# HugoVuach/Dense-linear-app

Measured on AMD Instinct MI355X. Metric: fp64 TFLOP/s for NxN SPD Cholesky (N^3/3 flops / factorisation time), higher is better.
Workload: dtype f64

## Files before the change

dense_linear_app_amd/csrc/kernels.hip:

```cpp
#include "cholmi_internal.h"

#include <type_traits>

#if defined(__HIP_DEVICE_COMPILE__) && !defined(__gfx950__)
#error "libcholmi's kernels target gfx950 (MI355X) only: build with --offload-arch=gfx950"
#endif

namespace cholmi {

typedef double d4_t __attribute__((ext_vector_type(4)));
typedef double d2_t __attribute__((ext_vector_type(2)));
typedef float f4_t __attribute__((ext_vector_type(4)));

template <typename T>
struct Tr;
template <>
struct Tr<double> {
  using acc_t = d4_t;
  using vec_t = d2_t;
  static constexpr int EPV = 2;
  static __device__ __forceinline__ acc_t mfma(double a, double b, acc_t c) {
    return __builtin_amdgcn_mfma_f64_16x16x4f64(a, b, c, 0, 0, 0);
  }
  static __device__ __forceinline__ int drow(int lane, int reg) { return (lane >> 4) + 4 * reg; }
// ... 84 lines not shown
  __syncthreads();
  const int nk = K / BK;
  for (int kt = 0; kt < nk; ++kt) {
    const int cur = kt & 1;
    if (kt + 1 < nk) gload((kt + 1) * BK);
    T af[4], bf[4];
#pragma unroll
    for (int ks = 0; ks < BK / 4; ++ks) {
      const int kk = ks * 4 + (lane >> 4);
#pragma unroll
      for (int a = 0; a < 4; ++a) af[a] = sm.a[cur][kk][wr * 64 + a * 16 + (lane & 15)];
#pragma unroll
      for (int b = 0; b < 4; ++b) bf[b] = sm.b[cur][kk][wc * 64 + b * 16 + (lane & 15)];
      if (ks == BK / 4 - 1 && kt + 1 < nk) lstore(cur ^ 1);
#pragma unroll
      for (int a = 0; a < 4; ++a)
#pragma unroll
        for (int b = 0; b < 4; ++b) acc[a][b] = Tr<T>::mfma(bf[b], af[a], acc[a][b]);
    }
    __syncthreads();
  }
}

__device__ __forceinline__ int cu_slot() {
  const unsigned hw = __builtin_amdgcn_s_getreg(4 | (0 << 6) | (31 << 11));
  const unsigned xcc = __builtin_amdgcn_s_getreg(20 | (0 << 6) | (3 << 11));
  return (int)(((((xcc & 7u) * 8u + ((hw >> 13) & 7u)) * 2u + ((hw >> 12) & 1u)) * 16u) + ((hw >> 8) & 15u));
}
struct GuestOnCu {
  int *slot;
  __device__ __forceinline__ explicit GuestOnCu(int *tab) : slot(nullptr) {
    if (tab) {
      slot = tab + cu_slot();
      if (threadIdx.x == 0) __hip_atomic_fetch_add(slot, 1, __ATOMIC_RELAXED, __HIP_MEMORY_SCOPE_AGENT);
    }
  }
  __device__ __forceinline__ void leave() {
    if (slot && threadIdx.x == 0) __hip_atomic_fetch_add(slot, -1, __ATOMIC_RELAXED, __HIP_MEMORY_SCOPE_AGENT);
  }
};
__device__ __forceinline__ void yield_to_guest(const int *slot) {
  for (int spin = 0; spin < 4000; ++spin) {
    if (__hip_atomic_load(slot, __ATOMIC_RELAXED, __HIP_MEMORY_SCOPE_AGENT) == 0) break;
    __builtin_amdgcn_s_sleep(20);
  }
}

__device__ __forceinline__ void sem_wait(const int *sem, int target, int *fail) {
  if (sem) {
    if (threadIdx.x == 0) {
      bool ok = false;
      for (int i = 0; i < (1 << 25); ++i) {
        if (__hip_atomic_load(sem, __ATOMIC_RELAXED, __HIP_MEMORY_SCOPE_AGENT) >= target) {
          ok = true;
          break;
        }
        __builtin_amdgcn_s_sleep(8);
      }
      __builtin_amdgcn_fence(__ATOMIC_ACQUIRE, "agent");
      asm volatile("s_waitcnt vmcnt(0)" ::: "memory");
      if (!ok && fail) atomicExch(fail, 0x7ffffffe);
    }
    __syncthreads();
  }
}
__device__ __forceinline__ void sem_signal(int *sem) {
  if (sem) {
    __syncthreads();
    if (threadIdx.x == 0) {
      __builtin_amdgcn_fence(__ATOMIC_RELEASE, "agent");
      asm volatile("s_waitcnt vmcnt(0)" ::: "memory");
      __hip_atomic_fetch_add(sem, 1, __ATOMIC_RELAXED, __HIP_MEMORY_SCOPE_AGENT);
    }
  }
}

__device__ __forceinline__ double load_sc1(const double *p) { return __hip_atomic_load(p, __ATOMIC_RELAXED, __HIP_MEMORY_SCOPE_AGENT); }
__device__ __forceinline__ float load_sc1(const float *p) { return __hip_atomic_load(p, __ATOMIC_RELAXED, __HIP_MEMORY_SCOPE_AGENT); }
__device__ __forceinline__ void store_sc1(double *p, double v) { __hip_atomic_store(p, v, __ATOMIC_RELAXED, __HIP_MEMORY_SCOPE_AGENT); }
__device__ __forceinline__ void store_sc1(float *p, float v) { __hip_atomic_store(p, v, __ATOMIC_RELAXED, __HIP_MEMORY_SCOPE_AGENT); }
__device__ __forceinline__ void store_pair_sc1(double *p, double a, double b) {
  d2_t v = {a, b};
  asm volatile("global_store_dwordx4 %0, %1, off sc1" ::"v"(p), "v"(v) : "memory");
}
__device__ __forceinline__ void store_pair_sc1(float *p, float a, float b) {
  typedef float f2_t __attribute__((ext_vector_type(2)));
  f2_t v = {a, b};
  asm volatile("global_store_dwordx2 %0, %1, off sc1" ::"v"(p), "v"(v) : "memory");
}

__device__ __forceinline__ void dbg_mark(unsigned long long *dbg, int tag, int step, unsigned long long t0) {
  if (dbg && threadIdx.x == 0) {
    const unsigned long long slot = atomicAdd(dbg, 1ull);
    if (slot < 1000) {
      unsigned long long *p = dbg + 1 + 8 * slot;
      p[0] = t0;
      p[1] = __builtin_amdgcn_s_memrealtime();
      p[2] = (unsigned long long)tag;
      p[3] = (unsigned long long)step;
    }
  }
}

__global__ void k_sem_probe_wait(const int *sem, int *result) {
  int ok = 2;
  for (int i = 0; i < 20000; ++i) {
    if (__hip_atomic_load(sem, __ATOMIC_RELAXED, __HIP_MEMORY_SCOPE_AGENT) >= 1) {
      ok = 1;
      break;
    }
    __builtin_amdgcn_s_sleep(8);
  }
  *result = ok;
}
__global__ void k_sem_probe_set(int *sem) { sem_signal(sem); }

__global__ void k_sem_gate(const int *sem, int target, int *fail) { sem_wait(sem, target, fail); }
extern int g_poll_max_wgs;
inline bool poll_in_kernel(hipStream_t s, const int *sem, int target, int *fail, long wgs) {
  if (!sem) return false;
  if (wgs <= g_poll_max_wgs) return true;
  k_sem_gate<<<1, 64, 0, s>>>(sem, target, fail);
  return false;
}

template <typename T>
struct alignas(16) SmemP {
  T a[2][BK][MACRO];
  T b[2][BK][MACRO];
};

template <typename T>
__device__ __forceinline__ void nt_kloop_paired(const T *__restrict__ A, int lda,
                                                const T *__restrict__ B, int ldb, int K, Acc<T> &acc,
                                                SmemP<T> &sm, const int *yslot = nullptr) {
  using vec_t = typename Tr<T>::vec_t;
  constexpr int EPV = Tr<T>::EPV;
  constexpr int NG = 4 / EPV;
  const int t = threadIdx.x, lane = t & 63, w = t >> 6, wr = w & 1, wc = w >> 1;
  constexpr int PIECES = BK * MACRO * (int)sizeof(T) / 1024;
  constexpr int EPP = 1024 / (int)sizeof(T);
  auto dma = [&](int buf, int k0) {
#pragma unroll
    for (int q = 0; q < PIECES / 4; ++q) {
      const int piece = q * 4 + w;
      const int e = piece * EPP + lane * EPV;
      const int kk = e / MACRO, r = e % MACRO;
      __builtin_amdgcn_global_load_lds(
          (const __attribute__((address_space(1))) void *)(A + r + (size_t)(k0 + kk) * lda),
          (__attribute__((address_space(3))) void *)(&sm.a[buf][0][0] + piece * EPP), 16, 0, 0);
      __builtin_amdgcn_global_load_lds(
          (const __attribute__((address_space(1))) void *)(B + r + (size_t)(k0 + kk) * ldb),
          (__attribute__((address_space(3))) void *)(&sm.b[buf][0][0] + piece * EPP), 16, 0, 0);
    }
  };
  vec_t fa[2][NG], fb[2][NG];
  const int arow = wr * 64 + EPV * (lane & 15), brow = wc * 64 + EPV * (lane & 15), kq = lane >> 4;
  auto fread = [&](int set, int cur, int ks) {
#pragma unroll
    for (int g = 0; g < NG; ++g) {
      fa[set][g] = *reinterpret_cast<const vec_t *>(&sm.a[cur][ks * 4 + kq][arow + g * 16 * EPV]);
      fb[set][g] = *reinterpret_cast<const vec_t *>(&sm.b[cur][ks * 4 + kq][brow + g * 16 * EPV]);
    }
  };

  dma(0, 0);
  __syncthreads();
  const int nk = K / BK;
  for (int kt = 0; kt < nk; ++kt) {
    const int cur = kt & 1;
    int guest = 0;
    if (yslot) guest = __hip_atomic_load(yslot, __ATOMIC_RELAXED, __HIP_MEMORY_SCOPE_AGENT);
    fread(0, cur, 0);
    if (kt + 1 < nk) dma(cur ^ 1, (kt + 1) * BK);
#pragma unroll
    for (int ks = 0; ks < BK / 4; ++ks) {
      __builtin_amdgcn_sched_barrier(0);
      acc[0][0] = Tr<T>::mfma(fb[ks & 1][0][0], fa[ks & 1][0][0], acc[0][0]);
      __builtin_amdgcn_sched_barrier(0);
      if (ks + 1 < BK / 4) fread((ks + 1) & 1, cur, ks + 1);
      __builtin_amdgcn_sched_barrier(0);
#pragma unroll
      for (int a = 0; a < 4; ++a)
#pragma unroll
        for (int b = 0; b < 4; ++b)
          if (a + b > 0)
            acc[a][b] = Tr<T>::mfma(fb[ks & 1][b / EPV][b % EPV], fa[ks & 1][a / EPV][a % EPV], acc[a][b]);
      __builtin_amdgcn_sched_barrier(0);
    }
    if (yslot && __builtin_amdgcn_readfirstlane(guest) != 0) yield_to_guest(yslot);
    __syncthreads();
  }
}

template <typename T, bool LOWER>
__device__ __forceinline__ void nt_epilogue_paired_impl(T *__restrict__ C, int ldc, Acc<T> &acc,
                                                        T alpha, T beta) {
  using vec_t = typename Tr<T>::vec_t;
  constexpr int EPV = Tr<T>::EPV, NG = 4 / EPV;
  const int t = threadIdx.x, lane = t & 63, w = t >> 6, wr = w & 1, wc = w >> 1;
  const int m0 = wr * 64 + EPV * (lane & 15);
#pragma unroll
  for (int b = 0; b < 4; ++b) {
    vec_t cv[4][NG];
#pragma unroll
    for (int r = 0; r < 4; ++r) {
      const int n = wc * 64 + (b / EPV) * 16 * EPV + EPV * Tr<T>::drow(lane, r) + b % EPV;
      const T *col = C + (size_t)n * ldc + m0;
#pragma unroll
      for (int g = 0; g < NG; ++g)
        if (beta != T(0)) cv[r][g] = *reinterpret_cast<const vec_t *>(col + g * 16 * EPV);
    }
#pragma unroll
    for (int r = 0; r < 4; ++r)
#pragma unroll
      for (int g = 0; g < NG; ++g)
#pragma unroll
        for (int e = 0; e < EPV; ++e) {
          const T v = alpha * acc[g * EPV + e][b][r];
          cv[r][g][e] = (beta != T(0)) ? v + beta * cv[r][g][e] : v;
        }
#pragma unroll
    for (int r = 0; r < 4; ++r) {
      const int n = wc * 64 + (b / EPV) * 16 * EPV + EPV * Tr<T>::drow(lane, r) + b % EPV;
      T *col = C + (size_t)n * ldc + m0;
#pragma unroll
      for (int g = 0; g < NG; ++g) {
        const int m = m0 + g * 16 * EPV;
        if (!LOWER || m >= n) {
          *reinterpret_cast<vec_t *>(col + g * 16 * EPV) = cv[r][g];
        } else {
#pragma unroll
          for (int e = 0; e < EPV; ++e)
            if (m + e >= n) col[g * 16 * EPV + e] = cv[r][g][e];
        }
      }
    }
  }
}

template <typename T>
__device__ __forceinline__ void nt_epilogue_paired(T *__restrict__ C, int ldc, Acc<T> &acc, T alpha,
                                                   T beta, bool lower) {
  if (lower)
    nt_epilogue_paired_impl<T, true>(C, ldc, acc, alpha, beta);
  else
    nt_epilogue_paired_impl<T, false>(C, ldc, acc, alpha, beta);
}

template <typename T>
__device__ __forceinline__ const T *panel_tile(const PanelRef &pan, int i, long bsiz) {
  const int p = i % pan.P;
  return reinterpret_cast<const T *>(pan.base[p]) + (long)(i / pan.P - pan.first[p]) * bsiz;
}

struct BlockMap {
  int2 ij;
  int mi, mj;
};
__device__ __forceinline__ bool map_update_block(const int2 *__restrict__ list, int na, int offb, int nb,
                                                 int nbm, int blocks_a, int unit, BlockMap &out, int b = -1) {
  if (b < 0) b = blockIdx.x;
  if (na == 0 && nb == 1) {
    int macro = b, mj = 0;
    while (macro >= nbm - mj) {
      macro -= nbm - mj;
      ++mj;
    }
    out.ij = list[offb];
    out.mj = mj;
    out.mi = mj + macro;
    return true;
  }
  if (b < blocks_a) {
    const int MT = nbm * nbm;
    const int x = b & 7, s = b >> 3;
    const int lin = ((s / unit) * 8 + x) * unit + s % unit;
    if (lin >= na * MT) return false;
    const int t = lin / MT, macro = lin - t * MT;
    out.ij = list[t];
    out.mi = macro % nbm;
    out.mj = macro / nbm;
    return true;
  }
  b -= blocks_a;
  const int MTd = nbm * (nbm + 1) / 2;
  const int ua = (na * nbm * nbm + unit - 1) / unit;
  const int x = ((b & 7) + 8 - ua % 8) & 7, s = b >> 3;
  const int lin = ((s / unit) * 8 + x) * unit + s % unit;
  if (lin >= nb * MTd) return false;
  const int t = lin / MTd;
  int macro = lin - t * MTd;
  out.ij = list[offb + t];
  int mj = 0;
  while (macro >= nbm - mj) {
    macro -= nbm - mj;
    ++mj;
  }
  out.mj = mj;
  out.mi = mj + macro;
  return true;
}

template <typename T, int MODE>
__device__ __forceinline__ void nt_kloop_w8(const T *__restrict__ A, int lda, const T *__restrict__ B, int ldb,
                                            int K, typename Tr<T>::acc_t (&acc)[4][2], SmemP<T> &sm,
                                            const int *yslot) {
  static_assert(sizeof(T) == 8, "fp64 only");
  using vec_t = typename Tr<T>::vec_t;
  const int t = threadIdx.x, lane = t & 63, w = t >> 6, wr = w & 1, wc = w >> 1, i = lane & 15, q = lane >> 4;
  constexpr int PIECES = BK * MACRO * (int)sizeof(T) / 1024, EPP = 1024 / (int)sizeof(T);
  auto dma_piece = [&](int buf, int k0, int p) {
    const int piece = p * 8 + w;
    const int e = piece * EPP + lane * 2;
    const int kk = e / MACRO, r = e % MACRO;
    __builtin_amdgcn_global_load_lds(
        (const __attribute__((address_space(1))) void *)(A + r + (size_t)(k0 + kk) * lda),
        (__attribute__((address_space(3))) void *)(&sm.a[buf][0][0] + piece * EPP), 16, 0, 0);
    __builtin_amdgcn_global_load_lds(
        (const __attribute__((address_space(1))) void *)(B + r + (size_t)(k0 + kk) * ldb),
        (__attribute__((address_space(3))) void *)(&sm.b[buf][0][0] + piece * EPP), 16, 0, 0);
  };
  auto dma = [&](int buf, int k0) {
#pragma unroll
    for (int p = 0; p < PIECES / 8; ++p) dma_piece(buf, k0, p);
  };
  static_assert(PIECES / 8 == 2, "two pieces per operand per wave and slice");
  vec_t fa[2][2], fb[2];
  const int arow = wr * 64 + 2 * i, brow = wc * 32 + 2 * i;
  if (MODE & 2) {
    if (w >= 4) __builtin_amdgcn_s_setprio(1);
  }
  auto fread = [&](int set, int cur, int ks) {
#pragma unroll
    for (int g = 0; g < 2; ++g) fa[set][g] = *reinterpret_cast<const vec_t *>(&sm.a[cur][ks * 4 + q][arow + 32 * g]);
    fb[set] = *reinterpret_cast<const vec_t *>(&sm.b[cur][ks * 4 + q][brow]);
  };
  dma(0, 0);
  __syncthreads();
  const int nk = K / BK;
  for (int kt = 0; kt < nk; ++kt) {
    const int cur = kt & 1;
    int guest = 0;
    if (yslot) guest = __hip_atomic_load(yslot, __ATOMIC_RELAXED, __HIP_MEMORY_SCOPE_AGENT);
    fread(0, cur, 0);
    if (!(MODE & 1) && kt + 1 < nk) dma(cur ^ 1, (kt + 1) * BK);
#pragma unroll
    for (int ks = 0; ks < BK / 4; ++ks) {
      __builtin_amdgcn_sched_barrier(0);
      acc[0][0] = Tr<T>::mfma(fb[ks & 1][0], fa[ks & 1][0][0], acc[0][0]);
      __builtin_amdgcn_sched_barrier(0);
      if (ks + 1 < BK / 4) fread((ks + 1) & 1, cur, ks + 1);
      if ((MODE & 1) && ks < 2 && kt + 1 < nk) dma_piece(cur ^ 1, (kt + 1) * BK, ks);
      __builtin_amdgcn_sched_barrier(0);
#pragma unroll
      for (int a = 0; a < 4; ++a)
#pragma unroll
        for (int b = 0; b < 2; ++b)
          if (a + b > 0) acc[a][b] = Tr<T>::mfma(fb[ks & 1][b], fa[ks & 1][a >> 1][a & 1], acc[a][b]);
      __builtin_amdgcn_sched_barrier(0);
    }
    if (yslot && __builtin_amdgcn_readfirstlane(guest) != 0) yield_to_guest(yslot);
    __syncthreads();
  }
}

template <typename T, bool OOP>
__device__ __forceinline__ void w8_epilogue(const T *Cin, T *Cout, int ld,
                                            typename Tr<T>::acc_t (&acc)[4][2], bool lower) {
  using vec_t = typename Tr<T>::vec_t;
  const int t = threadIdx.x, lane = t & 63, w = t >> 6, wr = w & 1, wc = w >> 1, i = lane & 15, q = lane >> 4;
  const int m0 = wr * 64 + 2 * i;
#pragma unroll
  for (int b = 0; b < 2; ++b) {
    vec_t cv[4][2];
#pragma unroll
    for (int r = 0; r < 4; ++r)
#pragma unroll
      for (int g = 0; g < 2; ++g)
        cv[r][g] = *reinterpret_cast<const vec_t *>(Cin + (long)(wc * 32 + 2 * (q + 4 * r) + b) * ld + m0 + 32 * g);
#pragma unroll
    for (int r = 0; r < 4; ++r) {
      const int n = wc * 32 + 2 * (q + 4 * r) + b;
      T *col = Cout + (long)n * ld;
#pragma unroll
      for (int g = 0; g < 2; ++g) {
        const int m = m0 + 32 * g;
        vec_t v = cv[r][g];
        if (OOP && lower && m < n) {
          if (m + 1 >= n) v[1] -= acc[2 * g + 1][b][r];
          *reinterpret_cast<vec_t *>(col + m) = v;
          continue;
        }
        v[0] -= acc[2 * g][b][r];
        v[1] -= acc[2 * g + 1][b][r];
        if (!lower || m >= n) {
          *reinterpret_cast<vec_t *>(col + m) = v;
        } else {
          if (m + 1 >= n) col[m + 1] = v[1];
        }
      }
    }
    __builtin_amdgcn_sched_barrier(0);
  }
}

template <typename T, int MODE>
__device__ __forceinline__ void trail_update_w8_block(const LocalMat &C, const int2 *__restrict__ list, int na, int offb,
                                                      int nb, int blocks_a, const PanelRef &pan, int nbm, int unit,
                                                      const int *ytab, const PanelRef &pan2, int npan, SmemP<T> &sm, int b) {
  using vec_t = typename Tr<T>::vec_t;
  BlockMap bm;
  if (!map_update_block(list, na, offb, nb, nbm, blocks_a, unit, bm, b)) return;
  const int2 ij = bm.ij;
  const int mi = bm.mi, mj = bm.mj;
  const bool lower = (ij.x == ij.y) && mi == mj;
  T *Cp = reinterpret_cast<T *>(C.base) + ((long)(ij.x / C.P) + (long)(ij.y / C.Q) * C.lmt) * C.bsiz +
          mi * MACRO + (long)mj * MACRO * C.mb;
  typename Tr<T>::acc_t acc[4][2];
#pragma unroll
  for (int a = 0; a < 4; ++a)
#pragma unroll
    for (int b = 0; b < 2; ++b)
#pragma unroll
      for (int r = 0; r < 4; ++r) acc[a][b][r] = T(0);
  const int *yslot = ytab ? ytab + cu_slot() : nullptr;
  nt_kloop_w8<T, MODE>(panel_tile<T>(pan, ij.x, C.bsiz) + mi * MACRO, C.mb, panel_tile<T>(pan, ij.y, C.bsiz) + mj * MACRO,
                 C.mb, C.mb, acc, sm, yslot);
  if (npan > 1)
    nt_kloop_w8<T, MODE>(panel_tile<T>(pan2, ij.x, C.bsiz) + mi * MACRO, C.mb,
                   panel_tile<T>(pan2, ij.y, C.bsiz) + mj * MACRO, C.mb, C.mb, acc, sm, yslot);
  w8_epilogue<T, false>(Cp, Cp, C.mb, acc, lower);
}

template <typename T, int MODE>
__global__ __launch_bounds__(512, 4) void k_trail_update_w8(LocalMat C, const int2 *__restrict__ list, int na,
                                                             int offb, int nb, int blocks_a, PanelRef pan, int nbm,
                                                             int unit, const int *ytab, PanelRef pan2, int npan) {
  __shared__ SmemP<T> sm;
  trail_update_w8_block<T, MODE>(C, list, na, offb, nb, blocks_a, pan, nbm, unit, ytab, pan2, npan, sm, (int)blockIdx.x);
}

constexpr int BKF = 32;
struct alignas(16) SmemF {
  float a[2][BKF][MACRO];
  float b[2][BKF][MACRO];
};
typedef float f2_t __attribute__((ext_vector_type(2)));

__device__ __forceinline__ void nt_kloop_w8f(const float *__restrict__ A, int lda, const float *__restrict__ B,
                                             int ldb, int K, f4_t (&acc)[4][2], SmemF &sm, const int *yslot) {
  const int t = threadIdx.x, lane = t & 63, w = t >> 6, wr = w & 1, wc = w >> 1, i = lane & 15, q = lane >> 4;
  constexpr int PIECES = BKF * MACRO * 4 / 1024, EPP = 256;
  auto dma = [&](int buf, int k0) {
#pragma unroll
    for (int p = 0; p < PIECES / 8; ++p) {
      const int piece = p * 8 + w;
      const int e = piece * EPP + lane * 4;
      const int kk = e / MACRO, r = e % MACRO;
      __builtin_amdgcn_global_load_lds(
          (const __attribute__((address_space(1))) void *)(A + r + (size_t)(k0 + kk) * lda),
          (__attribute__((address_space(3))) void *)(&sm.a[buf][0][0] + piece * EPP), 16, 0, 0);
      __builtin_amdgcn_global_load_lds(
          (const __attribute__((address_space(1))) void *)(B + ((r + 32 * (kk & 1)) & (MACRO - 1)) + (size_t)(k0 + kk) * ldb),
          (__attribute__((address_space(3))) void *)(&sm.b[buf][0][0] + piece * EPP), 16, 0, 0);
    }
  };
  f4_t fa[2];
  f2_t fb[2];
  const int arow = wr * 64 + 4 * i, brow = (wc * 32 + 2 * i - 32 * (q & 1)) & (MACRO - 1);
  auto fread = [&](int set, int cur, int ks) {
    fa[set] = *reinterpret_cast<const f4_t *>(&sm.a[cur][ks * 4 + q][arow]);
    fb[set] = *reinterpret_cast<const f2_t *>(&sm.b[cur][ks * 4 + q][brow]);
  };
  dma(0, 0);
  __syncthreads();
  const int nk = K / BKF;
  for (int kt = 0; kt < nk; ++kt) {
    const int cur = kt & 1;
    int guest = 0;
    if (yslot) guest = __hip_atomic_load(yslot, __ATOMIC_RELAXED, __HIP_MEMORY_SCOPE_AGENT);
    fread(0, cur, 0);
    if (kt + 1 < nk) dma(cur ^ 1, (kt + 1) * BKF);
#pragma unroll
    for (int ks = 0; ks < BKF / 4; ++ks) {
      __builtin_amdgcn_sched_barrier(0);
      acc[0][0] = Tr<float>::mfma(fb[ks & 1][0], fa[ks & 1][0], acc[0][0]);
      __builtin_amdgcn_sched_barrier(0);
      if (ks + 1 < BKF / 4) fread((ks + 1) & 1, cur, ks + 1);
      __builtin_amdgcn_sched_barrier(0);
#pragma unroll
      for (int a = 0; a < 4; ++a)
#pragma unroll
        for (int b = 0; b < 2; ++b)
          if (a + b > 0) acc[a][b] = Tr<float>::mfma(fb[ks & 1][b], fa[ks & 1][a], acc[a][b]);
      __builtin_amdgcn_sched_barrier(0);
    }
    if (yslot && __builtin_amdgcn_readfirstlane(guest) != 0) yield_to_guest(yslot);
    __syncthreads();
  }
}

template <bool OOP>
__device__ __forceinline__ void w8f_epilogue(const float *Cin, float *Cout, int ld, f4_t (&acc)[4][2], bool lower) {
  const int t = threadIdx.x, lane = t & 63, w = t >> 6, wr = w & 1, wc = w >> 1, i = lane & 15, q = lane >> 4;
  const int m0 = wr * 64 + 4 * i;
  f4_t cv[2][4];
#pragma unroll
  for (int b = 0; b < 2; ++b)
#pragma unroll
    for (int r = 0; r < 4; ++r)
      cv[b][r] = *reinterpret_cast<const f4_t *>(Cin + (long)(wc * 32 + 2 * (4 * q + r) + b) * ld + m0);
#pragma unroll
  for (int b = 0; b < 2; ++b)
#pragma unroll
    for (int r = 0; r < 4; ++r) {
      const int n = wc * 32 + 2 * (4 * q + r) + b;
      float *col = Cout + (long)n * ld;
      f4_t v = cv[b][r];
      if (OOP && lower && m0 < n) {
#pragma unroll
        for (int a = 0; a < 4; ++a)
          if (m0 + a >= n) v[a] -= acc[a][b][r];
        *reinterpret_cast<f4_t *>(col + m0) = v;
        continue;
      }
#pragma unroll
      for (int a = 0; a < 4; ++a) v[a] -= acc[a][b][r];
      if (!lower || m0 >= n) {
        *reinterpret_cast<f4_t *>(col + m0) = v;
      } else {
#pragma unroll
        for (int a = 0; a < 4; ++a)
          if (m0 + a >= n) col[m0 + a] = v[a];
      }
    }
}

__global__ __launch_bounds__(512, 4) void k_trail_update_w8f(LocalMat C, const int2 *__restrict__ list, int na,
                                                              int offb, int nb, int blocks_a, PanelRef pan, int nbm,
                                                              int unit, const int *ytab, PanelRef pan2, int npan) {
  __shared__ SmemF sm;
  BlockMap bm;
  if (!map_update_block(list, na, offb, nb, nbm, blocks_a, unit, bm)) return;
  const int2 ij = bm.ij;
  const int mi = bm.mi, mj = bm.mj;
  const bool lower = (ij.x == ij.y) && mi == mj;
  float *Cp = reinterpret_cast<float *>(C.base) + ((long)(ij.x / C.P) + (long)(ij.y / C.Q) * C.lmt) * C.bsiz +
              mi * MACRO + (long)mj * MACRO * C.mb;
  f4_t acc[4][2];
#pragma unroll
  for (int a = 0; a < 4; ++a)
#pragma unroll
    for (int b = 0; b < 2; ++b)
#pragma unroll
      for (int r = 0; r < 4; ++r) acc[a][b][r] = 0.f;
  const int *yslot = ytab ? ytab + cu_slot() : nullptr;
  nt_kloop_w8f(panel_tile<float>(pan, ij.x, C.bsiz) + mi * MACRO, C.mb,
               panel_tile<float>(pan, ij.y, C.bsiz) + mj * MACRO, C.mb, C.mb, acc, sm, yslot);
  if (npan > 1)
    nt_kloop_w8f(panel_tile<float>(pan2, ij.x, C.bsiz) + mi * MACRO, C.mb,
                 panel_tile<float>(pan2, ij.y, C.bsiz) + mj * MACRO, C.mb, C.mb, acc, sm, yslot);
  w8f_epilogue<false>(Cp, Cp, C.mb, acc, lower);
}

__device__ __forceinline__ bool map_ptr_block(int n, int nbm, int unit, int &t, int &mi, int &mj) {
  const int b = blockIdx.x, x = b & 7, sidx = b >> 3, MT = nbm * nbm;
  const long lin = ((long)(sidx / unit) * 8 + x) * unit + sidx % unit;
  if (lin >= (long)n * MT) return false;
  t = (int)(lin / MT);
  const int macro = (int)(lin - (long)t * MT);
  mi = macro % nbm;
  mj = macro / nbm;
  return true;
}
template <typename T>
__device__ __forceinline__ void copy_block_512(const T *cin, T *cout, int ld) {
  constexpr int EPV = 16 / (int)sizeof(T), VPC = MACRO / EPV;
  for (int e = threadIdx.x; e < MACRO * VPC; e += 512) {
    const int c = e / VPC, r = (e % VPC) * EPV;
    *reinterpret_cast<uint4 *>(cout + r + (long)c * ld) = *reinterpret_cast<const uint4 *>(cin + r + (long)c * ld);
  }
}
template <typename T, int MODE>
__global__ __launch_bounds__(512, 4) void k_update_ptrs_w8(const T *const *__restrict__ cin, const T *const *__restrict__ ap,
                                                            const T *const *__restrict__ bp, T *const *__restrict__ cout,
                                                            int n, int mb, int nbm, int unit, const int *ytab) {
  __shared__ SmemP<T> sm;
  int t, mi, mj;
  if (!map_ptr_block(n, nbm, unit, t, mi, mj)) return;
  const T *A = ap[t], *B = bp[t];
  const bool syrk = B == nullptr;
  const long off = mi * MACRO + (long)mj * MACRO * mb;
  const T *Ci = cin[t] + off;
  T *Co = cout[t] + off;
  if (syrk && mi < mj) {
    copy_block_512<T>(Ci, Co, mb);
    return;
  }
  if (syrk) B = A;
  typename Tr<T>::acc_t acc[4][2];
#pragma unroll
  for (int a = 0; a < 4; ++a)
#pragma unroll
    for (int b = 0; b < 2; ++b)
#pragma unroll
      for (int r = 0; r < 4; ++r) acc[a][b][r] = T(0);
  const int *yslot = ytab ? ytab + cu_slot() : nullptr;
  nt_kloop_w8<T, MODE>(A + mi * MACRO, mb, B + mj * MACRO, mb, mb, acc, sm, yslot);
  w8_epilogue<T, true>(Ci, Co, mb, acc, syrk && mi == mj);
}
__global__ __launch_bounds__(512, 4) void k_update_ptrs_w8f(const float *const *__restrict__ cin, const float *const *__restrict__ ap,
                                                             const float *const *__restrict__ bp, float *const *__restrict__ cout,
                                                             int n, int mb, int nbm, int unit, const int *ytab) {
  __shared__ SmemF sm;
  int t, mi, mj;
  if (!map_ptr_block(n, nbm, unit, t, mi, mj)) return;
  const float *A = ap[t], *B = bp[t];
  const bool syrk = B == nullptr;
  const long off = mi * MACRO + (long)mj * MACRO * mb;
  const float *Ci = cin[t] + off;
  float *Co = cout[t] + off;
  if (syrk && mi < mj) {
    copy_block_512<float>(Ci, Co, mb);
    return;
  }
  if (syrk) B = A;
  f4_t acc[4][2];
#pragma unroll
  for (int a = 0; a < 4; ++a)
#pragma unroll
    for (int b = 0; b < 2; ++b)
#pragma unroll
      for (int r = 0; r < 4; ++r) acc[a][b][r] = 0.f;
  const int *yslot = ytab ? ytab + cu_slot() : nullptr;
  nt_kloop_w8f(A + mi * MACRO, mb, B + mj * MACRO, mb, mb, acc, sm, yslot);
  w8f_epilogue<true>(Ci, Co, mb, acc, syrk && mi == mj);
}

template <typename T>
__global__ __launch_bounds__(256, 2) void k_panel_solve(T *tiles, long bsiz, int mb, int nbm, int r0,
                                                        int s, const T *__restrict__ winv, T alpha,
                                                        int *ytab, const int *wait_sem = nullptr,
                                                        int wait_target = 0, int *fail = nullptr,
                                                        int *head_sem = nullptr) {
  __shared__ SmemP<T> sm;
  sem_wait(wait_sem, wait_target, fail);
  GuestOnCu guest(ytab);
  __builtin_amdgcn_s_setprio(2);
  const int nr = nbm - r0;
  const int tix = blockIdx.x / nr, r = r0 + blockIdx.x % nr;
  T *Ap = tiles + (long)tix * bsiz + r * MACRO + (long)s * MACRO * mb;
  const T *Bp = winv + (long)s * MACRO * MACRO;
  Acc<T> acc;
  acc_zero<T>(acc);
  nt_kloop_paired<T>(Ap, mb, Bp, MACRO, MACRO, acc, sm);
  nt_epilogue_paired<T>(Ap, mb, acc, alpha, T(0), false);
  guest.leave();
  if (tix == 0) sem_signal(head_sem);
}

template <typename T>
__global__ __launch_bounds__(256, 2) void k_panel_update(T *tiles, long bsiz, int mb, int nbm, int s,
                                                         const T *__restrict__ lkk, T beta, int *ytab,
                                                         const int *wait_sem = nullptr, int wait_target = 0,
                                                         int *fail = nullptr) {
  __shared__ SmemP<T> sm;
  sem_wait(wait_sem, wait_target, fail);
  GuestOnCu guest(ytab);
  __builtin_amdgcn_s_setprio(2);
  const int nc = nbm - 1 - s;
  int b = blockIdx.x;
  const int c = s + 1 + b % nc;
  b /= nc;
  const int r = b % nbm, tix = b / nbm;
  T *tile = tiles + (long)tix * bsiz;
  const T *Ap = tile + r * MACRO + (long)s * MACRO * mb;
  const T *Bp = lkk + c * MACRO + (long)s * MACRO * mb;
  T *Cp = tile + r * MACRO + (long)c * MACRO * mb;
  Acc<T> acc;
  acc_zero<T>(acc);
  nt_kloop_paired<T>(Ap, mb, Bp, mb, MACRO, acc, sm);
  nt_epilogue_paired<T>(Cp, mb, acc, T(-1), beta, false);
  guest.leave();
}

constexpr int SK = 32;
template <typename T, int ROWS>
struct SmallImg {
  T v[SK][ROWS + 16];
};
template <typename T, int ROWS>
__device__ __forceinline__ void small_gload(const T *__restrict__ P, int ld, int k0, T (&r)[ROWS * SK / 256]) {
#pragma unroll
  for (int q = 0; q < ROWS * SK / 256; ++q) {
    const int e = threadIdx.x + 256 * q;
    r[q] = P[(e % ROWS) + (long)(k0 + e / ROWS) * ld];
  }
}
template <typename T, int ROWS>
__device__ __forceinline__ void small_lstore(SmallImg<T, ROWS> &img, const T (&r)[ROWS * SK / 256]) {
#pragma unroll
  for (int q = 0; q < ROWS * SK / 256; ++q) {
    const int e = threadIdx.x + 256 * q;
    img.v[e / ROWS][e % ROWS] = r[q];
  }
}
template <typename T, int RA, int RB>
__device__ __forceinline__ void small_mma(const SmallImg<T, RA> &ia, const SmallImg<T, RB> &ib, int i0, int j0,
                                          typename Tr<T>::acc_t (&acc)[2][2]) {
  const int lane = threadIdx.x & 63, lo = lane & 15, kq = lane >> 4;
#pragma unroll
  for (int ks = 0; ks < SK / 4; ++ks) {
    const int k = 4 * ks + kq;
    T af[2], bf[2];
#pragma unroll
    for (int a = 0; a < 2; ++a) af[a] = ia.v[k][i0 + 16 * a + lo];
#pragma unroll
    for (int b = 0; b < 2; ++b) bf[b] = ib.v[k][j0 + 16 * b + lo];
#pragma unroll
    for (int a = 0; a < 2; ++a)
#pragma unroll
      for (int b = 0; b < 2; ++b) acc[a][b] = Tr<T>::mfma(bf[b], af[a], acc[a][b]);
  }
}

template <typename T>
__global__ __launch_bounds__(256, 2) void k_solve_small(T *tiles, long bsiz, int mb, int nbm, int r0, int s,
                                                        const T *__restrict__ winv, T alpha, int *ytab,
                                                        const int *wait_sem = nullptr, int wait_target = 0,
                                                        int *fail = nullptr, int *head_sem = nullptr) {
  __shared__ SmallImg<T, 32> ia;
  __shared__ SmallImg<T, MACRO> ib;
  sem_wait(wait_sem, wait_target, fail);
  GuestOnCu guest(ytab);
  __builtin_amdgcn_s_setprio(2);
  const int per_tile = 4 * (nbm - r0);
  const int tix = blockIdx.x / per_tile, slab = blockIdx.x % per_tile;
  T *Ap = tiles + (long)tix * bsiz + (long)r0 * MACRO + 32 * slab + (long)s * MACRO * mb;
  const T *Bp = winv + (long)s * MACRO * MACRO;
  const int lane = threadIdx.x & 63, w = threadIdx.x >> 6, lo = lane & 15;
  T ra[32 * SK / 256], rb[MACRO * SK / 256];
  typename Tr<T>::acc_t acc[2][2];
#pragma unroll
  for (int a = 0; a < 2; ++a)
#pragma unroll
    for (int b = 0; b < 2; ++b)
#pragma unroll
      for (int r = 0; r < 4; ++r) acc[a][b][r] = T(0);
  small_gload<T, 32>(Ap, mb, 0, ra);
  small_gload<T, MACRO>(Bp, MACRO, 0, rb);
  for (int ph = 0; ph < MACRO / SK; ++ph) {
    small_lstore<T, 32>(ia, ra);
    small_lstore<T, MACRO>(ib, rb);
    __syncthreads();
    if (ph + 1 < MACRO / SK) {
      small_gload<T, 32>(Ap, mb, (ph + 1) * SK, ra);
      small_gload<T, MACRO>(Bp, MACRO, (ph + 1) * SK, rb);
    }
    small_mma<T, 32, MACRO>(ia, ib, 0, 32 * w, acc);
    __syncthreads();
  }
#pragma unroll
  for (int a = 0; a < 2; ++a)
#pragma unroll
    for (int b = 0; b < 2; ++b)
#pragma unroll
      for (int r = 0; r < 4; ++r)
        Ap[16 * a + lo + (long)(32 * w + 16 * b + Tr<T>::drow(lane, r)) * mb] = alpha * acc[a][b][r];
  guest.leave();
  if (tix == 0) sem_signal(head_sem);
}

template <typename T>
__global__ __launch_bounds__(256, 2) void k_small_update(T *C, long ldc, const T *__restrict__ A,
                                                        const T *__restrict__ B, long ldab, int K, int *ytab,
                                                        int full, long zc, long za, int *signal_sem = nullptr,
                                                        const int *wait_sem = nullptr, int wait_target = 0,
                                                        int *fail = nullptr) {
  __shared__ SmallImg<T, 64> ia, ib;
  const int r64 = blockIdx.x, c64 = blockIdx.y;
  if (!full && c64 > r64) return;
  C += blockIdx.z * zc;
  A += blockIdx.z * za;
  const T *Ap = A + 64 * r64;
  const T *Bp = B + 64 * c64;
  T *Cp = C + 64 * r64 + 64 * c64 * ldc;
  const int lane = threadIdx.x & 63, w = threadIdx.x >> 6, lo = lane & 15;
  const int i0 = 32 * (w & 1), j0 = 32 * (w >> 1);
  T ra[64 * SK / 256], rb[64 * SK / 256];
  typename Tr<T>::acc_t acc[2][2];
  T cv[2][2][4];
#pragma unroll
  for (int a = 0; a < 2; ++a)
#pragma unroll
    for (int b = 0; b < 2; ++b)
#pragma unroll
      for (int r = 0; r < 4; ++r) {
        acc[a][b][r] = T(0);
        cv[a][b][r] = Cp[(i0 + 16 * a + lo) + (long)(j0 + 16 * b + Tr<T>::drow(lane, r)) * ldc];
      }
  sem_wait(wait_sem, wait_target, fail);
  GuestOnCu guest(ytab);
  __builtin_amdgcn_s_setprio(2);
  small_gload<T, 64>(Ap, (int)ldab, 0, ra);
  small_gload<T, 64>(Bp, (int)ldab, 0, rb);
  const int nph = K / SK;
  for (int ph = 0; ph < nph; ++ph) {
    small_lstore<T, 64>(ia, ra);
    small_lstore<T, 64>(ib, rb);
    __syncthreads();
    if (ph + 1 < nph) {
      small_gload<T, 64>(Ap, (int)ldab, (ph + 1) * SK, ra);
      small_gload<T, 64>(Bp, (int)ldab, (ph + 1) * SK, rb);
    }
    small_mma<T, 64, 64>(ia, ib, i0, j0, acc);
    __syncthreads();
  }
  const bool dg = !full && (r64 == c64);
#pragma unroll
  for (int a = 0; a < 2; ++a)
#pragma unroll
    for (int b = 0; b < 2; ++b)
#pragma unroll
      for (int r = 0; r < 4; ++r) {
        const int i = i0 + 16 * a + lo, j = j0 + 16 * b + Tr<T>::drow(lane, r);
        if (!dg || i >= j) Cp[i + (long)j * ldc] = cv[a][b][r] - acc[a][b][r];
      }
  guest.leave();
  sem_signal(signal_sem);
}

template <typename T>
struct IntileLds {
  union {
    struct {
      SmallImg<T, 32> a;
      SmallImg<T, MACRO> b;
    } sv;
    struct {
      SmallImg<T, 64> a, b;
    } up;
  };
};
template <typename T>
__global__ __launch_bounds__(256, 2) void k_intile_step(T *tile, int mb, int nbm, int s, const T *__restrict__ winv,
                                                        int *ytab, int *cnt, int *fail) {
  __shared__ IntileLds<T> L;
  const int nr = nbm - 1 - s, nsolve = 4 * nr;
  const int lane = threadIdx.x & 63, w = threadIdx.x >> 6, lo = lane & 15;
  typename Tr<T>::acc_t acc[2][2];
#pragma unroll
  for (int a = 0; a < 2; ++a)
#pragma unroll
    for (int b = 0; b < 2; ++b)
#pragma unroll
      for (int r = 0; r < 4; ++r) acc[a][b][r] = T(0);
  if ((int)blockIdx.x < nsolve) {
    GuestOnCu guest(ytab);
    __builtin_amdgcn_s_setprio(2);
    T *Ap = tile + (long)(s + 1) * MACRO + 32 * (int)blockIdx.x + (long)s * MACRO * mb;
    const T *Bp = winv + (long)s * MACRO * MACRO;
    T ra[32 * SK / 256], rb[MACRO * SK / 256];
    small_gload<T, 32>(Ap, mb, 0, ra);
    small_gload<T, MACRO>(Bp, MACRO, 0, rb);
    for (int ph = 0; ph < MACRO / SK; ++ph) {
      small_lstore<T, 32>(L.sv.a, ra);
      small_lstore<T, MACRO>(L.sv.b, rb);
      __syncthreads();
      if (ph + 1 < MACRO / SK) {
        small_gload<T, 32>(Ap, mb, (ph + 1) * SK, ra);
        small_gload<T, MACRO>(Bp, MACRO, (ph + 1) * SK, rb);
      }
      small_mma<T, 32, MACRO>(L.sv.a, L.sv.b, 0, 32 * w, acc);
      __syncthreads();
    }
#pragma unroll
    for (int a = 0; a < 2; ++a)
#pragma unroll
      for (int b = 0; b < 2; ++b)
#pragma unroll
        for (int r = 0; r < 4; ++r)
          Ap[16 * a + lo + (long)(32 * w + 16 * b + Tr<T>::drow(lane, r)) * mb] = acc[a][b][r];
    guest.leave();
    sem_signal(cnt);
    return;
  }
  int c64 = 0, left = (int)blockIdx.x - nsolve, len = 2 * nr;
  while (left >= len) {
    left -= len;
    --len;
// ... 1421 lines not shown
```

Before: 68.79.

## Replace double-buffered fp64 k-loop with a 4-stage LDS ring and per-stage barriers

Rewrites the fp64 NT k-loop of the trailing-update kernels so that, instead of two BK-deep buffers with a full __syncthreads per slice, it uses a four-slot ring of 8-deep stages in the same 64 KiB of LDS. Each wave issues one 1-KiB DMA per operand per stage, with precomputed pointers that advance by a stride, and waits on a partial vmcnt plus a raw s_barrier, so loads stay up to three stages ahead. The MODE-based DMA split is dropped, and the guest-yield poll now runs every two stages. An optional compile-time s_memtime stamping probe is also added. The aim is better overlap of global-to-LDS traffic with MFMA work, at the cost of more frequent barriers and subtler vmcnt accounting.

```diff
diff --git a/dense_linear_app_amd/csrc/kernels.hip b/dense_linear_app_amd/csrc/kernels.hip
--- a/dense_linear_app_amd/csrc/kernels.hip
+++ b/dense_linear_app_amd/csrc/kernels.hip
@@ -410,68 +410,148 @@
   return true;
 }
 
+constexpr int BKR = 8, NST = 4;
+template <typename T>
+struct alignas(16) SmemR {
+  T a[NST][BKR][MACRO];
+  T b[NST][BKR][MACRO];
+};
+static_assert(sizeof(SmemR<double>) == sizeof(SmemP<double>), "the ring takes the double buffer's 64 KiB");
+
+#ifdef CHOLMI_KLOOP_STAMPS
+constexpr int KST_WGS = 16, KST_STAGES = 64, KST_REC = 4 + 5 * KST_STAGES;
+__device__ unsigned long long g_kloop_stamps[KST_WGS * 8 * KST_REC];
+#define KST_ON_STAGE(s) (kst_on && (s) < KST_STAGES)
+#define KSTAMP(on, idx)                                                                    \
+  do {                                                                                     \
+    if (on) {                                                                              \
+      __builtin_amdgcn_sched_barrier(0);                                                   \
+      unsigned long long t_;                                                               \
+      asm volatile("s_memtime %0\n\ts_waitcnt lgkmcnt(0)" : "=s"(t_)::"memory");           \
+      if (lane == 0) kst[idx] = t_;                                                        \
+      __builtin_amdgcn_sched_barrier(0);                                                   \
+    }                                                                                      \
+  } while (0)
+#else
+#define KST_ON_STAGE(s) false
+#define KSTAMP(on, idx) \
+  do {                  \
+  } while (0)
+#endif
+
 template <typename T, int MODE>
 __device__ __forceinline__ void nt_kloop_w8(const T *__restrict__ A, int lda, const T *__restrict__ B, int ldb,
-                                            int K, typename Tr<T>::acc_t (&acc)[4][2], SmemP<T> &sm,
+                                            int K, typename Tr<T>::acc_t (&acc)[4][2], SmemR<T> &sm,
                                             const int *yslot) {
   static_assert(sizeof(T) == 8, "fp64 only");
+  static_assert(BKR * MACRO * (int)sizeof(T) == 8 * 1024, "one 1-KiB piece per operand, wave and stage");
   using vec_t = typename Tr<T>::vec_t;
   const int t = threadIdx.x, lane = t & 63, w = t >> 6, wr = w & 1, wc = w >> 1, i = lane & 15, q = lane >> 4;
-  constexpr int PIECES = BK * MACRO * (int)sizeof(T) / 1024, EPP = 1024 / (int)sizeof(T);
-  auto dma_piece = [&](int buf, int k0, int p) {
-    const int piece = p * 8 + w;
-    const int e = piece * EPP + lane * 2;
-    const int kk = e / MACRO, r = e % MACRO;
-    __builtin_amdgcn_global_load_lds(
-        (const __attribute__((address_space(1))) void *)(A + r + (size_t)(k0 + kk) * lda),
-        (__attribute__((address_space(3))) void *)(&sm.a[buf][0][0] + piece * EPP), 16, 0, 0);
-    __builtin_amdgcn_global_load_lds(
-        (const __attribute__((address_space(1))) void *)(B + r + (size_t)(k0 + kk) * ldb),
-        (__attribute__((address_space(3))) void *)(&sm.b[buf][0][0] + piece * EPP), 16, 0, 0);
+  const int wu = __builtin_amdgcn_readfirstlane(w);
+  const char *ga = reinterpret_cast<const char *>(A + (size_t)wu * lda);
+  const char *gb = reinterpret_cast<const char *>(B + (size_t)wu * ldb);
+  const size_t da = (size_t)BKR * lda * sizeof(T), db = (size_t)BKR * ldb * sizeof(T);
+  const unsigned lo = (unsigned)lane * 16u;
+  auto dma = [&](int slot) {
+    __builtin_amdgcn_global_load_lds((const __attribute__((address_space(1))) void *)(ga + lo),
+                                     (__attribute__((address_space(3))) void *)(&sm.a[slot][wu][0]), 16, 0, 0);
+    __builtin_amdgcn_global_load_lds((const __attribute__((address_space(1))) void *)(gb + lo),
+                                     (__attribute__((address_space(3))) void *)(&sm.b[slot][wu][0]), 16, 0, 0);
+    ga += da;
+    gb += db;
   };
-  auto dma = [&](int buf, int k0) {
-#pragma unroll
-    for (int p = 0; p < PIECES / 8; ++p) dma_piece(buf, k0, p);
-  };
-  static_assert(PIECES / 8 == 2, "two pieces per operand per wave and slice");
+  const int *poll = yslot ? yslot : reinterpret_cast<const int *>(A);
   vec_t fa[2][2], fb[2];
   const int arow = wr * 64 + 2 * i, brow = wc * 32 + 2 * i;
   if (MODE & 2) {
     if (w >= 4) __builtin_amdgcn_s_setprio(1);
   }
-  auto fread = [&](int set, int cur, int ks) {
-#pragma unroll
-    for (int g = 0; g < 2; ++g) fa[set][g] = *reinterpret_cast<const vec_t *>(&sm.a[cur][ks * 4 + q][arow + 32 * g]);
-    fb[set] = *reinterpret_cast<const vec_t *>(&sm.b[cur][ks * 4 + q][brow]);
+  auto fread = [&](int set, int slot, int ks) {
+#pragma unroll
+    for (int g = 0; g < 2; ++g) fa[set][g] = *reinterpret_cast<const vec_t *>(&sm.a[slot][ks * 4 + q][arow + 32 * g]);
+    fb[set] = *reinterpret_cast<const vec_t *>(&sm.b[slot][ks * 4 + q][brow]);
   };
-  dma(0, 0);
-  __syncthreads();
-  const int nk = K / BK;
-  for (int kt = 0; kt < nk; ++kt) {
-    const int cur = kt & 1;
-    int guest = 0;
-    if (yslot) guest = __hip_atomic_load(yslot, __ATOMIC_RELAXED, __HIP_MEMORY_SCOPE_AGENT);
-    fread(0, cur, 0);
-    if (!(MODE & 1) && kt + 1 < nk) dma(cur ^ 1, (kt + 1) * BK);
-#pragma unroll
-    for (int ks = 0; ks < BK / 4; ++ks) {
+  auto mfma_rest = [&](int set) {
+#pragma unroll
+    for (int a = 0; a < 4; ++a)
+#pragma unroll
+      for (int b = 0; b < 2; ++b)
+        if (a + b > 0) acc[a][b] = Tr<T>::mfma(fb[set][b], fa[set][a >> 1][a & 1], acc[a][b]);
+  };
+#ifdef CHOLMI_KLOOP_STAMPS
+  const bool kst_on = blockIdx.x < KST_WGS;
+  unsigned long long *kst = g_kloop_stamps + ((size_t)blockIdx.x * 8 + wu) * KST_REC;
+  if (kst_on && lane == 0) {
+    kst[0] = __builtin_amdgcn_s_memtime();
+    kst[1] = __builtin_amdgcn_s_memrealtime();
+  }
+  __builtin_amdgcn_s_waitcnt(0xC07F);
+#endif
+  constexpr int VMCNT0 = 0x0F70;
+  const int ns = K / BKR;
+  dma(0);
+  dma(1);
+  dma(2);
+  __builtin_amdgcn_s_waitcnt(VMCNT0 + 4);
+  asm volatile("s_barrier" ::: "memory");
+  fread(0, 0, 0);
+  auto quad = [&](int s0, auto more_c) {
+    constexpr bool MORE = decltype(more_c)::value;
+    int guest;
+    static_for<0, NST>([&](auto jc) {
+      constexpr int j = decltype(jc)::value;
+      const int s = s0 + j;
+      const bool st = KST_ON_STAGE(s);
+      (void)st;
+      (void)s;
+      KSTAMP(st, 4 + 5 * s + 0);
       __builtin_amdgcn_sched_barrier(0);
-      acc[0][0] = Tr<T>::mfma(fb[ks & 1][0], fa[ks & 1][0][0], acc[0][0]);
+      acc[0][0] = Tr<T>::mfma(fb[0][0], fa[0][0][0], acc[0][0]);
       __builtin_amdgcn_sched_barrier(0);
-      if (ks + 1 < BK / 4) fread((ks + 1) & 1, cur, ks + 1);
-      if ((MODE & 1) && ks < 2 && kt + 1 < nk) dma_piece(cur ^ 1, (kt + 1) * BK, ks);
+      fread(1, j, 1);
       __builtin_amdgcn_sched_barrier(0);
-#pragma unroll
-      for (int a = 0; a < 4; ++a)
-#pragma unroll
-        for (int b = 0; b < 2; ++b)
-          if (a + b > 0) acc[a][b] = Tr<T>::mfma(fb[ks & 1][b], fa[ks & 1][a >> 1][a & 1], acc[a][b]);
+      mfma_rest(0);
       __builtin_amdgcn_sched_barrier(0);
-    }
-    if (yslot && __builtin_amdgcn_readfirstlane(guest) != 0) yield_to_guest(yslot);
-    __syncthreads();
-  }
-}
+      KSTAMP(st, 4 + 5 * s + 2);
+      __builtin_amdgcn_s_waitcnt(VMCNT0 + ((j < 2 || MORE) ? 2 : 0));
+      if ((j & 1) && yslot && __builtin_amdgcn_readfirstlane(guest) != 0) yield_to_guest(yslot);
+      asm volatile("s_barrier" ::: "memory");
+      KSTAMP(st, 4 + 5 * s + 3);
+      KSTAMP(st, 4 + 5 * s + 4);
+      __builtin_amdgcn_sched_barrier(0);
+      acc[0][0] = Tr<T>::mfma(fb[1][0], fa[1][0][0], acc[0][0]);
+      __builtin_amdgcn_sched_barrier(0);
+      if (j < NST - 1 || MORE) fread(0, (j + 1) % NST, 0);
+      if (!(j & 1)) guest = __hip_atomic_load(poll, __ATOMIC_RELAXED, __HIP_MEMORY_SCOPE_AGENT);
+      if (j == 0 || MORE) dma((j + 3) % NST);
+      __builtin_amdgcn_sched_barrier(0);
+      KSTAMP(st, 4 + 5 * s + 1);
+      mfma_rest(1);
+      __builtin_amdgcn_sched_barrier(0);
+    });
+  };
+  int s0 = 0;
+  for (; s0 < ns - NST; s0 += NST) quad(s0, std::true_type{});
+  quad(s0, std::false_type{});
+#ifdef CHOLMI_KLOOP_STAMPS
+  if (kst_on && lane == 0) {
+    kst[2] = __builtin_amdgcn_s_memtime();
+    kst[3] = __builtin_amdgcn_s_memrealtime();
+  }
+#endif
+}
+#ifdef CHOLMI_KLOOP_STAMPS
+}
+extern "C" __attribute__((visibility("default"))) int chol_debug_kloop_stamps(unsigned long long *out, int n) {
+  const int all = cholmi::KST_WGS * 8 * cholmi::KST_REC;
+  if (n > all) n = all;
+  if (hipDeviceSynchronize() != hipSuccess ||
+      hipMemcpyFromSymbol(out, HIP_SYMBOL(cholmi::g_kloop_stamps), (size_t)n * sizeof(unsigned long long)) != hipSuccess)
+    return -1;
+  return n;
+}
+namespace cholmi {
+#endif
 
 template <typename T, bool OOP>
 __device__ __forceinline__ void w8_epilogue(const T *Cin, T *Cout, int ld,
@@ -516,7 +596,7 @@
 template <typename T, int MODE>
 __device__ __forceinline__ void trail_update_w8_block(const LocalMat &C, const int2 *__restrict__ list, int na, int offb,
                                                       int nb, int blocks_a, const PanelRef &pan, int nbm, int unit,
-                                                      const int *ytab, const PanelRef &pan2, int npan, SmemP<T> &sm, int b) {
+                                                      const int *ytab, const PanelRef &pan2, int npan, SmemR<T> &sm, int b) {
   using vec_t = typename Tr<T>::vec_t;
   BlockMap bm;
   if (!map_update_block(list, na, offb, nb, nbm, blocks_a, unit, bm, b)) return;
@@ -545,7 +625,7 @@
 __global__ __launch_bounds__(512, 4) void k_trail_update_w8(LocalMat C, const int2 *__restrict__ list, int na,
                                                              int offb, int nb, int blocks_a, PanelRef pan, int nbm,
                                                              int unit, const int *ytab, PanelRef pan2, int npan) {
-  __shared__ SmemP<T> sm;
+  __shared__ SmemR<T> sm;
   trail_update_w8_block<T, MODE>(C, list, na, offb, nb, blocks_a, pan, nbm, unit, ytab, pan2, npan, sm, (int)blockIdx.x);
 }
 
@@ -694,7 +774,7 @@
 __global__ __launch_bounds__(512, 4) void k_update_ptrs_w8(const T *const *__restrict__ cin, const T *const *__restrict__ ap,
                                                             const T *const *__restrict__ bp, T *const *__restrict__ cout,
                                                             int n, int mb, int nbm, int unit, const int *ytab) {
-  __shared__ SmemP<T> sm;
+  __shared__ SmemR<T> sm;
   int t, mi, mj;
   if (!map_ptr_block(n, nbm, unit, t, mi, mj)) return;
   const T *A = ap[t], *B = bp[t];
```

New measurement: 70.68 (median of 6 runs). +2.8%, better.
